# Jackz915/PackPPI

Measured on AMD Instinct MI355X. Metric: sampled residues/sec at 100 diffusion steps, higher is better.
Workload: dtype f32 (dense layers as split-f16: two f16 per operand, three f16 MFMAs per product, fp32 accumulate); 1 GPU; data/T1124_lig.pdb (L=739, 738 true residues), 1 complex per GPU; diffusion_steps=100, proximal=False, residues_per_gpu=738, residues_rank0=738, residues_total=738, mode=ode

## Files before the change

packppi_amd/csrc/pp_api.hip:

```cpp
#include <stdio.h>
#include <stdlib.h>

#include <algorithm>
#include <chrono>
#include <cmath>
#include <cstring>
#include <memory>
#include <new>
#include <string>
#include <vector>

#include "pp_internal.h"
#include "pp_pack.h"
#ifdef PP_EDGE_F16
#include "pp_rebalance.h"
#endif
#include "pp_topk_aten.h"

static thread_local std::string g_err;
void pp_set_error(const std::string &msg) { g_err = msg; }

extern "C" const char *pp_last_error(void) { return g_err.c_str(); }
extern "C" int pp_version(void) { return 101; }
#ifndef PP_BUILD_ID
// ... 310 lines not shown
        if (min_len < PP_TOP_K && min_len != max_len)
            FAIL(PP_ERR_UNSUPPORTED, "pp_complex_prepare_packed: complexes shorter than 32 residues must be prepared on their own");
    }
    if (!b->X || !b->residue_type || !b->BB_D)
        FAIL(PP_ERR_INVALID, "pp_complex_prepare: batch needs at least X, residue_type and BB_D");
    const bool net = plan->has_network;
    if (net && (!b->atom_mask || !b->residue_mask || !b->residue_index || !b->chain_indices || !b->BB_D_sincos ||
                !b->SC_D_mask || !b->chi_1pi_periodic_mask || !b->chi_2pi_periodic_mask))
        FAIL(PP_ERR_INVALID, "pp_complex_prepare: batch has a null tensor pointer");
    PP_HIP_CHECK(hipSetDevice(plan->device));
    std::unique_ptr<pp_ctx, CtxDeleter> owner(new (std::nothrow) pp_ctx());
    if (!owner) FAIL(PP_ERR_INVALID, "out of host memory");
    pp_ctx *c = owner.get();
    c->plan = plan;
    c->b = *b;
    c->packed = packed;
    c->B = packed ? n_seg : b->B;
    c->L = packed ? max_len : b->L;
    c->N = b->B * b->L;
    const int shortest = packed ? min_len : b->L;
    c->K = shortest < PP_TOP_K ? shortest : PP_TOP_K;
    c->shortest = shortest;
    const size_t N = c->N, K = c->K;
    struct Slot { void **p; size_t bytes; };
    std::vector<Slot> slots;
    size_t total = 0;
#define ALLOC(field, n) { const size_t bytes_ = (((n) ? (n) : 1) * sizeof(*c->field) + 255) & ~size_t(255);          \
                          slots.push_back({reinterpret_cast<void **>(&c->field), bytes_}); total += bytes_; }
    if (net) {
        ALLOC(eidx, N * K); ALLOC(mask_att, N * 32); ALLOC(frames, N * 12); ALLOC(bbpos, N * 15);
        ALLOC(hE0, N * K * 128); ALLOC(hE, N * K * 128); ALLOC(Znm, N * K * 128); ALLOC(Zem, N * K * 128); ALLOC(hV, N * 128); ALLOC(hV_alt, N * 128); ALLOC(S, N * 128); ALLOC(msum, N);
        ALLOC(ptsN, N * 48); ALLOC(PAn, N * 128); ALLOC(PCn, N * 128);
        ALLOC(ptsE, N * 48); ALLOC(PAe, N * 128); ALLOC(PCe, N * 128);
        ALLOC(score, N * 4); ALLOC(chi_tmp, N * 4);
        for (int k = 0; k < 2; k++) { ALLOC(live_rows[k], N + 2); ALLOC(live_mix[k], N); ALLOC(live_cnt[k], 1); }
    }
    ALLOC(xyz, N * 42); ALLOC(rec, N * 64); ALLOC(axes, N * 24); ALLOC(rec2, N * 64); ALLOC(axes2, N * 24); ALLOC(brad, N); ALLOC(per_res, N); ALLOC(dchi, N * 4);
    ALLOC(px, N * 4); ALLOC(pm, N * 4); ALLOC(pv, N * 4); ALLOC(pz, N * 4); ALLOC(pxeff, N * 4); ALLOC(pmask, N);
    const bool prox = c->B == 1 || packed;
    if (prox) { ALLOC(cand, (size_t)N * 4 * PP_CL_CAP); ALLOC(cand_cnt, N * 4); }
    ALLOC(scal, 64);
    ALLOC(sat, 4);
    ALLOC(seg, N);
    ALLOC(prox_part, (size_t)PP_PROX_CHUNK * N);
    if (prox) { ALLOC(prox_nrows, c->B); ALLOC(prox_seg, c->B); ALLOC(prox_inv, N); }
    if (prox) { ALLOC(obst_seg, c->B); ALLOC(obst_row, N); ALLOC(obst_cand, (size_t)N * PP_OB_CAP); ALLOC(obst_cnt, N); }
    ALLOC(sasa_row, N * 8);
    ALLOC(seg_off, (size_t)c->B + 1);
    ALLOC(rng_tab, N); ALLOC(rng_keys, c->B);
    c->max_steps = 1 << 20;
#undef ALLOC
    c->last_stream = static_cast<hipStream_t>(stream);
    {
        std::lock_guard<std::mutex> g(plan->pool_mutex);
        int best = -1;
        for (int i = 0; i < (int)plan->arena_pool.size(); i++)
            if (plan->arena_pool[i].bytes >= total && (best < 0 || plan->arena_pool[i].bytes < plan->arena_pool[best].bytes)) best = i;
        if (best >= 0) {
            const ArenaSlot sl = plan->arena_pool[best];
            plan->arena_pool.erase(plan->arena_pool.begin() + best);
            if (sl.stream != c->last_stream) (void)hipStreamSynchronize(sl.stream);
            c->arena = sl.p;
            c->arena_bytes = sl.bytes;
        }
    }
    if (!c->arena && hipMalloc(&c->arena, total) != hipSuccess) {
        c->arena = nullptr;
// ... 654 lines not shown
```

packppi_amd/csrc/pp_internal.h:

```cpp
#pragma once
#include <hip/hip_runtime.h>
#include <hip/hip_ext.h>
#include <cmath>
#include <vector>
#include <mutex>
#include <stdint.h>
#include <string>

#include "../../include/packppi_hip.h"

#if defined(PP_LAB) && !defined(PP_DIAG)
#define PP_DIAG
#endif
#if !defined(PP_LAB) &&                                                                                                       \
    (defined(PP_X_TS) || defined(PP_X_TS_FINE) || defined(PP_X_NOWLOAD) || defined(PP_X_E_NOMFMA) || defined(PP_X_NOSAT) ||      \
     defined(PP_WDEPTH) || defined(PP_WDEPTH_R1) || defined(PP_NXB_R1) || defined(PP_WGS2) || defined(PP_WGS) ||                 \
     defined(PP_NM_WGS2) ||                                                                                                  \
     defined(PP_LDS_PAD) || defined(PP_NO_FUSE_NM) || defined(PP_NU_DEPTH))
#error "PP_X_* / tuning switches compile laboratory variants (most give wrong results): add -DPP_LAB and build a TAGGED library (python -m packppi_amd.build --tag NAME -DPP_LAB -DPP_X_...)"
#endif
#ifdef PP_DIAG
#define PP_GETENV(name) getenv(name)
#else
#define PP_GETENV(name) ((const char *)nullptr)
// ... 76 lines not shown

struct StepParams {
    float temb[16];
    float c_ode;
    float w;
    float c_drift;
    float c_diff;
    float pad[12];
};

struct pp_ctx {
    pp_plan *plan;
    pp_batch b;
    int B, L, K, N;
    bool packed = false;
    int shortest = 0;
    int32_t *seg_off;
    int2 *seg;
    int32_t *eidx;
    float *mask_att;
    float *frames;
    float *bbpos;
    float *hE0;
    float *Znm, *Zem;
    float *hE;
    float *hV;
    float *hV_alt;
    float *S;
    float *msum;
    float *ptsN, *PAn, *PCn;
    float *ptsE, *PAe, *PCe;
    float *score;
    float *chi_tmp;
    void *arena = nullptr;
    size_t arena_bytes = 0;
    hipStream_t last_stream = nullptr;
    int max_steps;
    float *xyz;
    float *rec;
    float *axes;
    float *rec2, *axes2;
    float *brad;
    float *per_res;
    float *dchi;
    float *px, *pm, *pv, *pz, *pxeff;
    uint8_t *pmask;
    int32_t *cand;
    int32_t *cand_cnt;
    float *prox_part;
    int32_t *prox_nrows;
    float2 *prox_seg;
    float *prox_inv;
    float *scal;
    float4 *obst = nullptr;
    int obst_M = 0;
    int obst_cap = 0;
    int2 *obst_seg;
    int2 *obst_row;
    int32_t *obst_cand;
    int32_t *obst_cnt;
    float *sasa_row;
    pp_rng_row *rng_tab;
    uint64_t *rng_keys;
    bool rng_tab_set = false;
    int32_t *live_rows[2];
    int2 *live_mix[2];
// ... 134 lines not shown
    float *chi;
    int step, mode;
    const float *noise;
    const StepParams *cur;
    const StepParams *next;
    const PPRng *rng;
    const PPPin *pin;
};
pp_status pp_launch_node_update(pp_ctx *c, int layer, int last_mode, const NodeEval &ev, hipStream_t s);
pp_status pp_launch_edge_static(pp_ctx *c, hipStream_t s);
#ifdef PP_EDGE_F16
pp_status pp_launch_edge_embed_f16(pp_ctx *c, hipStream_t s);
#endif
pp_status pp_launch_node_message(pp_ctx *c, int layer, hipStream_t s);
bool pp_edge_fused();
pp_status pp_launch_edge_update(pp_ctx *c, int layer, bool keep_hE, hipStream_t s, const PPLive *live = nullptr);
pp_status pp_launch_atom14(pp_ctx *c, const float *chi, float *xyz, hipStream_t s);
pp_status pp_launch_clash(pp_ctx *c, const float *xyz, float *per_res, float *dchi, hipStream_t s, bool use_candidates = false);
pp_status pp_launch_proximal(pp_ctx *c, const float *chi, float lamda, int nsteps, float *traj,
                             float *chi_last, float *losses, hipStream_t s);
pp_status pp_launch_proximal_packed(pp_ctx *c, const float *chi, float lamda, int nsteps, bool norm_given, float *traj,
                                    float *chi_last, float *chi_accepted, float *losses, hipStream_t s,
                                    const uint8_t *fixed = nullptr, uint8_t *moved = nullptr);

pp_status pp_launch_guide_begin(pp_ctx *c, hipStream_t s);
pp_status pp_launch_guide_nudge(pp_ctx *c, float *chi, const uint8_t *fixed, float eta, float cap, double *trace, int n_schedule,
                                int j, hipStream_t s);

pp_status pp_launch_correct(pp_ctx *c, float *chi, const uint8_t *fixed, float snr, int j, int n_steps, const PPRng &rng,
                            double *trace, hipStream_t s);

void pp_edge_occupancy(int *node_msg, int *edge_upd);

#define PP_NU_MID 0
#define PP_NU_SCORE 1
#define PP_NU_STEP 2
```

packppi_amd/csrc/pp_node.hip:

```cpp
#include <string.h>

#include "pp_internal.h"
#include <utility>

PP_RANGE_COUNTER
PP_RANGE_READER(pp_node_range_hits)

#define NT 512
#ifndef PP_NODE_GROUPS
#define PP_NODE_GROUPS 1
#endif
#define NG PP_NODE_GROUPS
#define NB (4 * NG)

struct NodeArgs {
    int N;
    const float *rmask;
    const int64_t *rtype;
    const float *bb_sincos;
    const float *sc_mask;
    const uint8_t *m1pi, *m2pi;
    const float *frames;
    const float *embT, *emb_b, *emb_g, *emb_beta;
    float *hV, *S, *msum;
// ... 278 lines not shown
};

struct SmemU {
    _Float16 a_hi[16 * NU_S128], a_lo[16 * NU_S128];
    _Float16 b_hi[16 * NU_S128], b_lo[16 * NU_S128];
    _Float16 c_hi[16 * NU_S512], c_lo[16 * NU_S512];
    float stats[3][8][16][2];
    float pts[16][48];
    _Float16 e_hi[16 * NU_S32], e_lo[16 * NU_S32];
    float fr[16][12];
    float par[NU_P_LAST_TOTAL];
};

struct StepScalars {
    float c_ode, w, c_drift, c_diff;
};
struct TimeEmb {
    float v[16];
};

struct NUpdArgs {
    int N;
    const float *rmask;
    const int64_t *rtype;
    const float *bb_sincos;
    const float *sc_mask;
    const uint8_t *m1pi, *m2pi;
    const float *frames;
    const float *embT;
    const float *wstream, *params;
    const float *hV;
    float *hV_out;
    const float *S, *msum;
    float *ptsN, *PAn, *PCn, *ptsE, *PAe, *PCe, *score;
    unsigned *sat;
};

template <bool LAST>
__device__ constexpr int nu_slot_waves(int s) {
    if (!LAST) return s < 52 ? 8 : 3;
    return s < 36 ? 8 : s < 40 ? 4 : s < 46 ? 1 : s < 55 ? 8 : 2;
}

template <int CL>
__device__ __forceinline__ int nu_phys_slot(int s, int q) {
    if constexpr (CL == 1) return s;
    constexpr int NPS = 16 / CL;
    return s < 36 ? s : s < 36 + NPS ? s + NPS * q : s + (16 - NPS);
}
template <bool LAST, int CL>
__device__ constexpr int nu_logical_waves(int s) {
    if (CL == 1) return nu_slot_waves<LAST>(s);
    return s < 36 + 16 / CL ? 8 : 3;
}
__device__ __forceinline__ void gload_N(const nh8 *__restrict__ wq, int slot, AOpN &a) {
    int off = slot * 128;
    asm volatile("" : "+s"(off));
    const nh8 *p = wq + off;
    a.hi = p[0];
    a.lo = p[64];
}
#define MFMA_N(a, b, c) __builtin_amdgcn_mfma_f32_16x16x32_f16((a), (b), (c), 0, 0, 0)
__device__ __forceinline__ void mm3(const AOpN &a, const nh8 &bh, const nh8 &bl, nf4 &cH, nf4 &cL) {
    cH = MFMA_N(a.hi, bh, cH);
    cL = MFMA_N(a.hi, bl, cL);
    cL = MFMA_N(a.lo, bh, cL);
}
__device__ __forceinline__ nf4 fold(const nf4 &cH, const nf4 &cL) {
    return nf4{fmaf(cL[0], NU_INV_LO, cH[0]), fmaf(cL[1], NU_INV_LO, cH[1]), fmaf(cL[2], NU_INV_LO, cH[2]), fmaf(cL[3], NU_INV_LO, cH[3])};
}
__device__ __forceinline__ void ldB(const _Float16 *hi, const _Float16 *lo, int rowoff, int ks, nh8 &bh, nh8 &bl) {
    bh = *reinterpret_cast<const nh8 *>(hi + rowoff + 32 * ks);
    bl = *reinterpret_cast<const nh8 *>(lo + rowoff + 32 * ks);
}
__device__ __forceinline__ void split2(float x0, float x1, unsigned &hp, unsigned &lp) {
    unsigned a, b, c, d;
    float fa, fb;
    PP_RANGE(x0) PP_RANGE(x1)
    asm("v_cvt_f16_f32 %0, %1" : "=v"(a) : "v"(x0));
    asm("v_cvt_f16_f32 %0, %1" : "=v"(b) : "v"(x1));
    asm("v_cvt_f32_f16 %0, %1" : "=v"(fa) : "v"(a));
    asm("v_cvt_f32_f16 %0, %1" : "=v"(fb) : "v"(b));
    const float d0 = (x0 - fa) * PP_NU_LO_SCALE, d1 = (x1 - fb) * PP_NU_LO_SCALE;
    asm("v_cvt_f16_f32 %0, %1" : "=v"(c) : "v"(d0));
    asm("v_cvt_f16_f32 %0, %1" : "=v"(d) : "v"(d1));
    asm("v_pack_b32_f16 %0, %1, %2" : "=v"(hp) : "v"(a), "v"(b));
    asm("v_pack_b32_f16 %0, %1, %2" : "=v"(lp) : "v"(c), "v"(d));
// ... 14 lines not shown
}
__device__ __forceinline__ float xsum_g(float v) {
    v += __shfl_xor(v, 16);
    v += __shfl_xor(v, 32);
    return v;
}
__device__ __forceinline__ nf4 ln128(float (*st)[16][2], int wv, int r, int g, const nf4 &x, const nf4 &gain, const nf4 &beta) {
    const float mw = xsum_g((x[0] + x[1]) + (x[2] + x[3])) * (1.f / 16.f);
    const nf4 d = x - mw;
    const float qw = xsum_g(fmaf(d[0], d[0], d[1] * d[1]) + fmaf(d[2], d[2], d[3] * d[3]));
    if (g == 0) *reinterpret_cast<nf2 *>(st[wv][r]) = nf2{mw, qw};
    __syncthreads();
    float m8[8], msum = 0.f, qsum = 0.f;
#pragma unroll
    for (int v = 0; v < 8; v++) {
        const nf2 t = *reinterpret_cast<const nf2 *>(st[v][r]);
        m8[v] = t[0];
        msum += t[0];
        qsum += t[1];
    }
    const float mean = msum * 0.125f;
    float dm = 0.f;
#pragma unroll
    for (int v = 0; v < 8; v++) dm = fmaf(m8[v] - mean, m8[v] - mean, dm);
    const float var = fmaf(16.f, dm, qsum) * (1.f / 128.f);
    const float rstd = 1.f / sqrtf(var + 1e-5f);
    return (x - mean) * rstd * gain + beta;
}

#define NSTAGE_IF(k, OWN, ACCV, BODY)                                                                                  \
    {                                                                                                                  \
        __builtin_amdgcn_sched_barrier(0);                                                                             \
        if constexpr ((k) + NU_ND < NLOAD) {                                                           \
            constexpr int nw_ = nu_logical_waves<LAST, CL>((k) + NU_ND);                                               \
            if (nw_ == 8 || wv < nw_)                                                                                  \
                gload_N(wq, nu_phys_slot<CL>((k) + NU_ND, clq), AR[((k) + NU_ND) % NU_NRING]);                         \
        }                                                                                                              \
        if (OWN) {                                                                                                     \
            const AOpN &AK = AR[(k) % NU_NRING];                                                                       \
            BODY;                                                                                                      \
            asm volatile("" ::"v"(ACCV[0]));                                                                           \
        }                                                                                                              \
    }
#define NSTAGE(k, ACCV, BODY) NSTAGE_IF(k, true, ACCV, BODY)
#define NTILE4_IF(k0, OWN, cH, cL)                                     \
    NSTAGE_IF((k0) + 0, OWN, cH, mm3(AK, bh[0], bl[0], cH, cL))        \
    NSTAGE_IF((k0) + 1, OWN, cH, mm3(AK, bh[1], bl[1], cH, cL))        \
    NSTAGE_IF((k0) + 2, OWN, cH, mm3(AK, bh[2], bl[2], cH, cL))        \
    NSTAGE_IF((k0) + 3, OWN, cH, mm3(AK, bh[3], bl[3], cH, cL))
#define NTILE4(k0, cH, cL) NTILE4_IF(k0, true, cH, cL)
#define LDB4(HI, LO)                                                                  \
    _Pragma("unroll") for (int ks_ = 0; ks_ < 4; ks_++) ldB(HI, LO, r * NU_S128 + 8 * g, ks_, bh[ks_], bl[ks_]);
#define FOSTAGE(s)                                                                                   \
    NSTAGE(20 + (s), cH, {                                                                           \
        if constexpr ((s) + 1 < 16) ldB(sm.c_hi, sm.c_lo, r * NU_S512 + 8 * g, (s) + 1, fh[((s) + 1) & 1], fl[((s) + 1) & 1]); \
        mm3(AK, fh[(s) & 1], fl[(s) & 1], cH, cL);                                                   \
    })

template <int MODE, int NU_ND, int CL = 1, bool SEEDED = false, bool PINNED = false>
__global__ void __launch_bounds__(512)
k_node_update(NUpdArgs A, float *chi, int step, int sde, const float *noise, int embed_next, StepScalars sp, TimeEmb te_next, PPRng rng,
              PPPin pin) {
    static_assert(CL == 1 || MODE == PP_NU_MID, "only the middle layers have a split form");
    static_assert(!SEEDED || MODE == PP_NU_STEP, "only the reverse step draws noise");
    static_assert(!PINNED || SEEDED, "the pinned step is a seeded one: its fixed rows re-noise with the step's own draws");
    constexpr int NU_NRING = NU_ND + 1;
    constexpr bool LAST = MODE != PP_NU_MID;
    constexpr int NSLOT = LAST ? PP_NU_SLOTS_LAST : PP_NU_SLOTS_MID;
    constexpr int NLOAD = MODE == PP_NU_SCORE ? 46 : CL > 1 ? 36 + 16 / CL + 4 : NSLOT;
    const int clq = CL > 1 ? (int)(blockIdx.x % CL) : 0;
    constexpr int NPAR = LAST ? NU_P_LAST_TOTAL : NU_P_MID_TOTAL;
    extern __shared__ __attribute__((aligned(16))) char smem_raw[];
    SmemU &sm = *reinterpret_cast<SmemU *>(smem_raw);
    const int tid = threadIdx.x, lane = tid & 63, wv = __builtin_amdgcn_readfirstlane(tid >> 6);
    const int r = lane & 15, g = lane >> 4, N = A.N, n0 = (int)(blockIdx.x / CL) * 16;
    const int n = n0 + r, nc = n < N ? n : N - 1;
    const bool live = n < N;
    const int fc = 16 * wv + 4 * g;
    const float *par = sm.par;

    const int srow = tid >> 5, scol = (tid & 31) * 4, sn = n0 + srow < N ? n0 + srow : N - 1;
    const nf4 s4 = *reinterpret_cast<const nf4 *>(A.S + (size_t)sn * 128 + scol);
    const nf4 hv4 = *reinterpret_cast<const nf4 *>(A.hV + (size_t)nc * 128 + fc);
    const float ms = A.msum[nc], rm = A.rmask[nc];
    const nf4 zero4i = {0.f, 0.f, 0.f, 0.f};
    float chi1 = 0.f, scm1 = 0.f, nz1 = 0.f, nz2 = 0.f;
    unsigned char m1raw = 0, m2raw = 0;
    int rt = 0;
    pp_rng_row rrow = {0u, 0u, 0u, 0u};
    unsigned char fixraw = 0;
    float cref = 0.f;
    nf4 spv = zero4i;
    if constexpr (MODE == PP_NU_STEP) {
        spv = nf4{sp.c_ode, sp.w, sp.c_drift, sp.c_diff};
        chi1 = chi[(size_t)nc * 4 + g];
        scm1 = A.sc_mask[(size_t)nc * 4 + g];
        m1raw = A.m1pi[(size_t)nc * 4 + g];
        m2raw = A.m2pi[(size_t)nc * 4 + g];
        if constexpr (PINNED) {
            fixraw = pin.fixed[nc];
            cref = pin.chi_ref[(size_t)nc * 4 + g];
        }
        if constexpr (SEEDED) {
            rrow = rng.tab[nc];
        } else if (sde) {
            const size_t NN = (size_t)N * 4;
            const float *nz = noise + (size_t)step * 2 * NN + (size_t)nc * 4 + g;
            nz1 = nz[0];
            nz2 = nz[NN];
        }
        rt = (int)A.rtype[nc];
    }
    nf4 tailv = {0.f, 0.f, 0.f, 0.f};
    nf4 ev[4] = {tailv, tailv, tailv, tailv};
    const int erow = tid & 15, ern = n0 + erow < N ? n0 + erow : N - 1;
    const bool e_bb = MODE == PP_NU_STEP && tid >= 128 && tid < 144, e_te = MODE == PP_NU_STEP && tid >= 192 && tid < 208;
    {
        const int t48 = tid % 48, row = t48 / 3, rn = n0 + row < N ? n0 + row : N - 1;
        tailv = *reinterpret_cast<const nf4 *>(A.frames + (size_t)rn * 12 + 4 * (t48 - 3 * row));
    }
    nf2 bb0 = {0.f, 0.f}, bb1 = bb0, bb2 = bb0;
    if constexpr (MODE == PP_NU_STEP) {
        const nf2 *bp = reinterpret_cast<const nf2 *>(A.bb_sincos + (size_t)ern * 6);
        bb0 = bp[0]; bb1 = bp[1]; bb2 = bp[2];
    }
    constexpr int NPV = (NPAR / 4 + 511) / 512;
    nf4 pv[NPV];
#pragma unroll
// ... 52 lines not shown
        publish4(sm.e_hi, sm.e_lo, erow * NU_S32 + 16, nf4{ev[0][2], ev[0][3], ev[1][0], ev[1][1]});
        publish4(sm.e_hi, sm.e_lo, erow * NU_S32 + 20, nf4{ev[1][2], ev[1][3], ev[2][0], ev[2][1]});
        publish4(sm.e_hi, sm.e_lo, erow * NU_S32 + 24, nf4{ev[2][2], ev[2][3], ev[3][0], ev[3][1]});
        publish4(sm.e_hi, sm.e_lo, erow * NU_S32 + 28, nf4{ev[3][2], ev[3][3], 0.f, 0.f});
    }
    publish4(sm.a_hi, sm.a_lo, srow * NU_S128 + scol, s4);
    unsigned satrows = 0xffffu;
    if constexpr (MODE == PP_NU_STEP) {
        const unsigned long long bs = __ballot(scm1 != 0.f);
        const unsigned long long br = __ballot(rm != 0.f && (!PINNED || fixraw == 0));
        satrows = (unsigned)((bs | (bs >> 16) | (bs >> 32) | (bs >> 48)) & br & 0xffffull);
    }
    __syncthreads();

    nh8 bh[4], bl[4];
    nf4 cH, cL;
    float satm = 0.f;
    const nf4 zero4 = zero4i;
    LDB4(sm.a_hi, sm.a_lo)
    cH = zero4; cL = zero4;
    NTILE4(0, cH, cL)
    nf4 x = fold(cH, cL) + *reinterpret_cast<const nf4 *>(par + NU_P_OUTB + fc) * ms + hv4;
    const nf4 h1 = ln128(sm.stats[0], wv, r, g, x, *reinterpret_cast<const nf4 *>(par + NU_P_G0 + fc),
                         *reinterpret_cast<const nf4 *>(par + NU_P_B0 + fc));
    publish4(sm.b_hi, sm.b_lo, r * NU_S128 + fc, h1);
    __syncthreads();
    LDB4(sm.b_hi, sm.b_lo)
#define FFN_IN_TILE(c)                                                                                     \
    cH = zero4; cL = zero4;                                                                                \
    NTILE4(4 + 4 * (c), cH, cL)                                                                            \
    publish4(sm.c_hi, sm.c_lo, r * NU_S512 + 16 * (4 * wv + (c)) + 4 * g,                                  \
             relu_sat(fold(cH, cL) + *reinterpret_cast<const nf4 *>(par + NU_P_FIB + 16 * (4 * wv + (c)) + 4 * g), satm));
    FFN_IN_TILE(0) FFN_IN_TILE(1) FFN_IN_TILE(2) FFN_IN_TILE(3)
    const bool satrow = (satrows >> r) & 1u;
    if (!(satm < 65504.f) && satrow) atomicOr(A.sat, 2u);
    __syncthreads();
    nh8 fh[2], fl[2];
    ldB(sm.c_hi, sm.c_lo, r * NU_S512 + 8 * g, 0, fh[0], fl[0]);
    cH = zero4; cL = zero4;
    FOSTAGE(0) FOSTAGE(1) FOSTAGE(2) FOSTAGE(3) FOSTAGE(4) FOSTAGE(5) FOSTAGE(6) FOSTAGE(7)
    FOSTAGE(8) FOSTAGE(9) FOSTAGE(10) FOSTAGE(11) FOSTAGE(12) FOSTAGE(13) FOSTAGE(14) FOSTAGE(15)
    x = fold(cH, cL) + *reinterpret_cast<const nf4 *>(par + NU_P_FOB + fc) + h1;
    const nf4 h2 = ln128(sm.stats[1], wv, r, g, x, *reinterpret_cast<const nf4 *>(par + NU_P_G1 + fc),
                         *reinterpret_cast<const nf4 *>(par + NU_P_B1 + fc)) * rm;
    if (live && clq == 0 && (MODE != PP_NU_STEP || !embed_next)) *reinterpret_cast<nf4 *>(A.hV_out + (size_t)n * 128 + fc) = h2;
    publish4(sm.a_hi, sm.a_lo, r * NU_S128 + fc, h2);
    __syncthreads();
    LDB4(sm.a_hi, sm.a_lo)

    if constexpr (!LAST) {
        constexpr int NPJ = 4 / CL;
#define NU_PROJ(i)                                                                                                     \
        if constexpr ((i) < NPJ) {                                                                                     \
            cH = zero4; cL = zero4;                                                                                    \
            NTILE4(36 + 4 * (i), cH, cL)                                                                               \
            const int pj = NPJ * clq + (i);                                                                            \
            float *dst = pj == 0 ? A.PAe : pj == 1 ? A.PCe : pj == 2 ? A.PAn : A.PCn;                                  \
            nf4 v = fold(cH, cL);                                                                                      \
            if (pj == 0) v = v + *reinterpret_cast<const nf4 *>(par + NU_P_PAE_B + fc);                                \
            else if (pj == 2) v = v + *reinterpret_cast<const nf4 *>(par + NU_P_PAN_B + fc);                           \
            if (live) *reinterpret_cast<nf4 *>(dst + (size_t)n * 128 + fc) = v;                                        \
        }
        NU_PROJ(0) NU_PROJ(1) NU_PROJ(2) NU_PROJ(3)
#undef NU_PROJ
        if (CL > 1 && clq != 0) return;
        cH = zero4; cL = zero4;
        NTILE4_IF(36 + 4 * NPJ, wv < 3, cH, cL)
// ... 27 lines not shown
        __syncthreads();
        const bool w0 = wv == 0;
        {
            nh8 dh[2], dl[2];
            if (w0) {
                ldB(sm.c_hi, sm.c_lo, r * NU_S512 + 8 * g, 0, dh[0], dl[0]);
                ldB(sm.c_hi, sm.c_lo, r * NU_S512 + 8 * g, 1, dh[1], dl[1]);
            }
            nf4 eH = zero4, eL = zero4;
            cH = zero4; cL = zero4;
            NSTAGE_IF(40, w0, cH, mm3(AK, dh[0], dl[0], cH, cL))
            NSTAGE_IF(41, w0, cH, mm3(AK, dh[1], dl[1], cH, cL))
            NSTAGE_IF(42, w0, eH, mm3(AK, dh[0], dl[0], eH, eL))
            NSTAGE_IF(43, w0, eH, mm3(AK, dh[1], dl[1], eH, eL))
            if (w0) {
                publish4(sm.c_hi, sm.c_lo, r * NU_S512 + 64 + 4 * g, relu_sat(fold(cH, cL) + *reinterpret_cast<const nf4 *>(par + NU_P_DB1 + 4 * g), satm));
                publish4(sm.c_hi, sm.c_lo, r * NU_S512 + 80 + 4 * g, relu_sat(fold(eH, eL) + *reinterpret_cast<const nf4 *>(par + NU_P_DB1 + 16 + 4 * g), satm));
                asm volatile("s_waitcnt lgkmcnt(0)" ::: "memory");
                ldB(sm.c_hi, sm.c_lo, r * NU_S512 + 8 * g, 2, dh[0], dl[0]);
            }
            cH = zero4; cL = zero4;
            NSTAGE_IF(44, w0, cH, mm3(AK, dh[0], dl[0], cH, cL))
            if (w0) {
                publish4(sm.c_hi, sm.c_lo, r * NU_S512 + 96 + 4 * g, relu_sat(fold(cH, cL) + *reinterpret_cast<const nf4 *>(par + NU_P_DB2 + 4 * g), satm));
                asm volatile("s_waitcnt lgkmcnt(0)" ::: "memory");
                ldB(sm.c_hi, sm.c_lo, r * NU_S512 + 8 * g, 3, dh[0], dl[0]);
            }
            cH = zero4; cL = zero4;
            NSTAGE_IF(45, w0, cH, mm3(AK, dh[0], dl[0], cH, cL))
        }
        if (w0) {
            if (!(satm < 65504.f) && satrow) atomicOr(A.sat, 2u);
            const nf4 sc = fold(cH, cL) + *reinterpret_cast<const nf4 *>(par + NU_P_DB3);
            if (g == 0 && live) *reinterpret_cast<nf4 *>(A.score + (size_t)n * 4) = sc;
            if constexpr (MODE == PP_NU_STEP) {
                const float s0 = __shfl(sc[0], r), s1 = __shfl(sc[1], r), s2 = __shfl(sc[2], r), s3 = __shfl(sc[3], r);
                const float sg = g == 0 ? s0 : g == 1 ? s1 : g == 2 ? s2 : s3;
                const float sp_c_ode = spv[0], sp_w = spv[1], sp_c_drift = spv[2], sp_c_diff = spv[3];
                const float sw = sg * sp_w;
#define NU_M1ON (PINNED ? m1raw == 1 : m1raw != 0)
                float yk = chi1;
                if (!sde) {
                    if (NU_M1ON || m2raw != 0) yk = chi1 + sp_c_ode * sw;
                } else {
                    if (NU_M1ON) yk = chi1 + (sp_c_drift * sw + sp_c_diff * nz1);
                    if (m2raw != 0) yk = yk + (sp_c_drift * sw + sp_c_diff * nz2);
                }
#undef NU_M1ON
                float y = wrap_pi(yk) * scm1;
                if constexpr (PINNED) {
                    if (m1raw == 2) y = chi1;
                }
                if (live) chi[(size_t)n * 4 + g] = y;
                if constexpr (PINNED) {
                    if (pin.traj != nullptr && live) pin.traj[(size_t)n * 4 + g] = y;
                }
                if (embed_next) {
                    unsigned hp, lp;
                    split2(sinf(y) * scm1, cosf(y) * scm1, hp, lp);
                    *reinterpret_cast<unsigned *>(sm.e_hi + r * NU_S32 + 6 + 2 * g) = hp;
                    *reinterpret_cast<unsigned *>(sm.e_lo + r * NU_S32 + 6 + 2 * g) = lp;
                }
            }
        }
        if constexpr (MODE != PP_NU_STEP) return;
        if (!embed_next) return;
        __syncthreads();
        nh8 eh, el;
        eh = *reinterpret_cast<const nh8 *>(sm.e_hi + r * NU_S32 + 8 * g);
        el = *reinterpret_cast<const nh8 *>(sm.e_lo + r * NU_S32 + 8 * g);
        cH = zero4; cL = zero4;
        NSTAGE(46, cH, mm3(AK, eh, el, cH, cL))
        const nf4 e0 = fold(cH, cL) + (*reinterpret_cast<const nf4 *>(par + NU_P_EMB_B + fc) + oh4);
        const nf4 h0 = ln128(sm.stats[2], wv, r, g, e0, *reinterpret_cast<const nf4 *>(par + NU_P_EMB_G + fc),
                             *reinterpret_cast<const nf4 *>(par + NU_P_EMB_BETA + fc));
        if (live) *reinterpret_cast<nf4 *>(A.hV_out + (size_t)n * 128 + fc) = h0;
        publish4(sm.b_hi, sm.b_lo, r * NU_S128 + fc, h0);
        __syncthreads();
        LDB4(sm.b_hi, sm.b_lo)
        cH = zero4; cL = zero4;
        NTILE4(47, cH, cL)
        if (live) *reinterpret_cast<nf4 *>(A.PAn + (size_t)n * 128 + fc) = fold(cH, cL) + *reinterpret_cast<const nf4 *>(par + NU_P_PAN0_B + fc);
        cH = zero4; cL = zero4;
        NTILE4(51, cH, cL)
        if (live) *reinterpret_cast<nf4 *>(A.PCn + (size_t)n * 128 + fc) = fold(cH, cL);
        if (wv < 2) {
            cH = zero4; cL = zero4;
            NTILE4(55, cH, cL)
            if (fc < 24) {
                const nf4 p = fold(cH, cL) + *reinterpret_cast<const nf4 *>(par + NU_P_PTS0_B + fc);
                *reinterpret_cast<nf4 *>(&sm.pts[r][fc]) = p;
                if (live) *reinterpret_cast<nf4 *>(A.ptsN + (size_t)n * 48 + fc) = p;
            }
        }
        __syncthreads();
        if (tid < 128) {
            const int q = tid >> 4, i = tid & 15, ni = n0 + i;
            if (ni < N) {
                const float *fr = sm.fr[i];
                const float px = sm.pts[i][3 * q], py = sm.pts[i][3 * q + 1], pz = sm.pts[i][3 * q + 2];
#pragma unroll
                for (int rr = 0; rr < 3; rr++)
                    A.ptsN[(size_t)ni * 48 + 24 + 3 * q + rr] = (fr[3 * rr] * px + fr[3 * rr + 1] * py + fr[3 * rr + 2] * pz) + fr[9 + rr];
            }
        }
    }
}

#ifndef PP_EDGE_F16
struct UpdW {
    const float *outT, *out_b;
    const float *g0, *b0, *g1, *b1;
    const float *ffn_inT, *ffn_in_b, *ffn_outT, *ffn_out_b;
    PreW pre_edge, pre_next;
    const float *d0_inT, *d0_in_b, *d0_outT, *d0_out_b, *d2_inT, *d2_in_b, *d2_outT, *d2_out_b;
};

struct WSet {
    float v[32];
};
template <int KL, int DST0 = 0>
// ... 345 lines not shown
}
static PreW make_pre(const pp_plan *p, int layer, bool edge) {
    const LayerOff &o = p->off.layer[layer];
    const LayerT &t = p->lt[layer];
    PreW w;
    w.ptsT = edge ? t.pts_edge_wT : t.pts_node_wT;
    w.pts_b = p->w + (edge ? o.pts_edge_b : o.pts_node_b);
    w.AT = edge ? t.em_A_T : t.nm_A_T;
    w.CT = edge ? t.em_C_T : t.nm_C_T;
    w.in_b = p->w + (edge ? o.em_in_b : o.nm_in_b);
    return w;
}

template <typename F>
struct NuInstance {
    int mode, depth, split;
    bool seeded, pinned;
    F fn;
};
typedef void (*nu_kernel_t)(NUpdArgs, float *, int, int, const float *, int, StepScalars, TimeEmb, PPRng, PPPin);
static const NuInstance<nu_kernel_t> nu_table[] = {
    {PP_NU_STEP, PP_NU_DEPTH_MULTI, 1, false, false, k_node_update<PP_NU_STEP, PP_NU_DEPTH_MULTI>},
    {PP_NU_SCORE, PP_NU_DEPTH_MULTI, 1, false, false, k_node_update<PP_NU_SCORE, PP_NU_DEPTH_MULTI>},
    {PP_NU_MID, PP_NU_DEPTH_MULTI, 1, false, false, k_node_update<PP_NU_MID, PP_NU_DEPTH_MULTI>},
    {PP_NU_STEP, PP_NU_DEPTH, 1, false, false, k_node_update<PP_NU_STEP, PP_NU_DEPTH>},
    {PP_NU_SCORE, PP_NU_DEPTH, 1, false, false, k_node_update<PP_NU_SCORE, PP_NU_DEPTH>},
    {PP_NU_MID, PP_NU_DEPTH, 1, false, false, k_node_update<PP_NU_MID, PP_NU_DEPTH>},
    {PP_NU_STEP, PP_NU_DEPTH_MULTI, 1, true, false, k_node_update<PP_NU_STEP, PP_NU_DEPTH_MULTI, 1, true>},
    {PP_NU_STEP, PP_NU_DEPTH, 1, true, false, k_node_update<PP_NU_STEP, PP_NU_DEPTH, 1, true>},
    {PP_NU_STEP, PP_NU_DEPTH_MULTI, 1, true, true, k_node_update<PP_NU_STEP, PP_NU_DEPTH_MULTI, 1, true, true>},
    {PP_NU_STEP, PP_NU_DEPTH, 1, true, true, k_node_update<PP_NU_STEP, PP_NU_DEPTH, 1, true, true>},
    {PP_NU_MID, PP_NU_DEPTH, 4, false, false, k_node_update<PP_NU_MID, PP_NU_DEPTH, 4>},
    {PP_NU_MID, PP_NU_DEPTH, 2, false, false, k_node_update<PP_NU_MID, PP_NU_DEPTH, 2>},
};
#ifndef PP_EDGE_F16
typedef void (*nv_kernel_t)(NodeArgs, UpdW, float *, int, int, const float *, int, PreW, StepScalars, TimeEmb, PPRng, PPPin);
static const NuInstance<nv_kernel_t> nv_table[] = {
    {PP_NU_MID, 0, 1, false, false, k_node_update_valu<PP_NU_MID>},
    {PP_NU_STEP, 0, 1, false, false, k_node_update_valu<PP_NU_STEP>},
    {PP_NU_SCORE, 0, 1, false, false, k_node_update_valu<PP_NU_SCORE>},
    {PP_NU_STEP, 0, 1, true, false, k_node_update_valu<PP_NU_STEP, true>},
    {PP_NU_STEP, 0, 1, true, true, k_node_update_valu<PP_NU_STEP, true, true>},
};
#endif
template <typename F, size_t n>
static F nu_find(const NuInstance<F> (&tab)[n], int mode, int depth, int split, bool seeded, bool pinned) {
    for (const NuInstance<F> &k : tab)
        if (k.mode == mode && k.depth == depth && k.split == split && k.seeded == seeded && k.pinned == pinned) return k.fn;
    return nullptr;
}
static int g_nu_cus = 0;
static pp_status node_attrs() {
    static bool done = false;
    if (!done) {
        PP_HIP_CHECK(hipFuncSetAttribute(reinterpret_cast<const void *>(k_node_embed),
                                         hipFuncAttributeMaxDynamicSharedMemorySize, (int)sizeof(Smem)));
        PP_HIP_CHECK(hipFuncSetAttribute(reinterpret_cast<const void *>(k_node_embed_rows),
                                         hipFuncAttributeMaxDynamicSharedMemorySize, (int)sizeof(Smem)));
        for (const auto &k : nu_table)
            PP_HIP_CHECK(hipFuncSetAttribute(reinterpret_cast<const void *>(k.fn), hipFuncAttributeMaxDynamicSharedMemorySize, (int)sizeof(SmemU)));
#ifndef PP_EDGE_F16
        for (const auto &k : nv_table)
            PP_HIP_CHECK(hipFuncSetAttribute(reinterpret_cast<const void *>(k.fn), hipFuncAttributeMaxDynamicSharedMemorySize, (int)sizeof(Smem)));
#endif
        int dev = 0;
        hipDeviceProp_t prop;
        if (hipGetDevice(&dev) == hipSuccess && hipGetDeviceProperties(&prop, dev) == hipSuccess) g_nu_cus = prop.multiProcessorCount;
        if (g_nu_cus <= 0) g_nu_cus = 256;
        done = true;
    }
    return PP_OK;
}

pp_status pp_launch_node_embed(pp_ctx *c, const float *chi, const StepParams &sp, hipStream_t s) {
    pp_status st = node_attrs();
    if (st != PP_OK) return st;
    NodeArgs A = make_args(c);
    PreW pre0 = make_pre(c->plan, 0, false);
    PP_LAUNCH(c, k_node_embed, dim3((c->N + NB - 1) / NB), dim3(NT), sizeof(Smem), s, A, pre0, chi, sp);
    PP_HIP_CHECK(hipGetLastError());
    return PP_OK;
}

pp_status pp_launch_node_embed_rows(pp_ctx *c, const float *chi, const float *t_rows, hipStream_t s) {
    pp_status st = node_attrs();
    if (st != PP_OK) return st;
    NodeArgs A = make_args(c);
    PreW pre0 = make_pre(c->plan, 0, false);
    TimeFreq fq;
    const float nemb = (float)(-(log(10000.0) / 7.0));
    for (int i = 0; i < 8; i++) fq.v[i] = expf((float)i * nemb);
    hipLaunchKernelGGL(k_node_embed_rows, dim3((c->N + NB - 1) / NB), dim3(NT), sizeof(Smem), s, A, pre0, chi, t_rows, fq);
    PP_HIP_CHECK(hipGetLastError());
    return PP_OK;
}

pp_status pp_launch_node_update(pp_ctx *c, int layer, int last_mode, const NodeEval &ev, hipStream_t s) {
    float *const chi = ev.chi;
    const int step = ev.step;
    const float *const noise = ev.noise;
    const StepParams *cur = last_mode != PP_NU_MID ? ev.cur : nullptr, *next = last_mode == PP_NU_STEP ? ev.next : nullptr;
    const bool pinned = ev.pin != nullptr && last_mode == PP_NU_STEP;
    if (pinned && (ev.rng == nullptr || ev.rng->tab == nullptr || ev.pin->fixed == nullptr || ev.pin->chi_ref == nullptr)) {
        pp_set_error("pp_launch_node_update: the pinned reverse step needs the rng table, fixed and chi_ref");
        return PP_ERR_INVALID;
    }
    const bool seeded = ev.rng != nullptr && ev.rng->tab != nullptr && last_mode == PP_NU_STEP && (ev.mode == PP_MODE_SDE || pinned);
    const PPRng rg = seeded ? *ev.rng : PPRng{nullptr, 0u, 0u};
    const PPPin pn = pinned ? *ev.pin : PPPin{nullptr, nullptr, nullptr, 0.f, 0};
    pp_status st0 = node_attrs();
    if (st0 != PP_OK) return st0;
    if ((last_mode == PP_NU_MID) != (layer < 2)) {
        pp_set_error("pp_launch_node_update: layers 0 and 1 are middle layers, layer 2 is the last one");
// ... 25 lines not shown
    TimeEmb te = {};
    if (cur) sp = {cur->c_ode, cur->w, cur->c_drift, cur->c_diff};
    if (next) memcpy(te.v, next->temb, sizeof(te.v));
#ifndef PP_EDGE_F16
    {
        static const bool f16_node = PP_GETENV("PP_NODE_F16") != nullptr;
        if (!f16_node) {
            const LayerOff &o = p->off.layer[layer];
            NodeArgs NA = make_args(c);
            UpdW W;
            W.outT = t.nm_out_T; W.out_b = p->w + o.nm_out_b;
            W.g0 = p->w + o.norm_g[0]; W.b0 = p->w + o.norm_b[0];
            W.g1 = p->w + o.norm_g[1]; W.b1 = p->w + o.norm_b[1];
            W.ffn_inT = t.nd_in_T; W.ffn_in_b = p->w + o.nd_in_b;
            W.ffn_outT = t.nd_out_T; W.ffn_out_b = p->w + o.nd_out_b;
            W.pre_edge = make_pre(p, layer, true);
            W.pre_next = make_pre(p, layer < 2 ? layer + 1 : 0, false);
            W.d0_inT = p->d0_in_T; W.d0_in_b = p->w + p->off.d0_in_b;
            W.d0_outT = p->d0_out_T; W.d0_out_b = p->w + p->off.d0_out_b;
            W.d2_inT = p->d2_in_T; W.d2_in_b = p->w + p->off.d2_in_b;
            W.d2_outT = p->d2_out_T; W.d2_out_b = p->w + p->off.d2_out_b;
            const PreW pre0 = make_pre(p, 0, false);
            const dim3 vgrid((c->N + NB - 1) / NB), vblock(NT);
            const nv_kernel_t kv = nu_find(nv_table, last_mode, 0, 1, seeded, pinned);
            if (!kv) FAIL(PP_ERR_UNSUPPORTED, "pp_launch_node_update: no such instance of k_node_update_valu");
            PP_LAUNCH(c, kv, vgrid, vblock, sizeof(Smem), s, NA, W, chi, step, sde, noise, embed_next, pre0, sp, te, rg, pn);
            PP_HIP_CHECK(hipGetLastError());
            return PP_OK;
        }
    }
#endif
    const bool multi = (int)grid.x > g_nu_cus;
    static const char *split_env = PP_GETENV("PP_NU_SPLIT");
    static const int split_max = split_env ? atoi(split_env) : 4;
    const int tiles = (int)grid.x;
    const int cl = last_mode != PP_NU_MID ? 1 : (split_max >= 4 && 4 * tiles <= g_nu_cus) ? 4 : (split_max >= 2 && 2 * tiles <= g_nu_cus) ? 2 : 1;
    if (cl > 1) {
        A.hV_out = c->hV_alt;
        std::swap(c->hV, c->hV_alt);
    }
    const nu_kernel_t kern = nu_find(nu_table, last_mode, cl > 1 || !multi ? PP_NU_DEPTH : PP_NU_DEPTH_MULTI, cl, seeded, pinned);
    if (!kern) FAIL(PP_ERR_UNSUPPORTED, "pp_launch_node_update: no such instance of k_node_update");
    PP_LAUNCH(c, kern, dim3(tiles * cl), block, sizeof(SmemU), s, A, chi, step, sde, noise, embed_next, sp, te, rg, pn);
    PP_HIP_CHECK(hipGetLastError());
    return PP_OK;
}

__global__ void k_rng_table(pp_rng_row *__restrict__ tab, int N, const int32_t *__restrict__ seg_off, int n_seg,
                            const uint64_t *__restrict__ keys) {
    const int n = blockIdx.x * blockDim.x + threadIdx.x;
    if (n >= N) return;
    const int ord = pp_seg_of_row(seg_off, n_seg, n);
    const int start = pp_seg_start(seg_off, ord, n);
    const uint64_t key = keys ? keys[ord] : (uint64_t)ord;
    pp_rng_row t;
    t.row = (uint32_t)(n - start);
    t.pad = 0u;
    t.ckey_lo = (uint32_t)key;
    t.ckey_hi = (uint32_t)(key >> 32);
    tab[n] = t;
}

__global__ void k_noise_seeded(const pp_rng_row *__restrict__ tab, int N, uint32_t seed_lo, uint32_t seed_hi, int step,
                               float *__restrict__ noise, uint32_t *__restrict__ words) {
    const int i = blockIdx.x * blockDim.x + threadIdx.x;
    if (i >= N * 4) return;
    const pp_rng_words w = pp_rng_draw(seed_lo, seed_hi, tab[i >> 2], i & 3, step);
    noise[i] = pp_rng_normal(w.o[0], w.o[1]);
    noise[(size_t)N * 4 + i] = pp_rng_normal(w.o[2], w.o[3]);
    if (words) *reinterpret_cast<uint4 *>(words + (size_t)i * 4) = make_uint4(w.o[0], w.o[1], w.o[2], w.o[3]);
}

// ... 118 lines not shown
```

Before: 63780 residues/s.

## Split the reverse-step node update across 2 or 3 workgroups per tile

Extends the cluster-split form of the node-update kernel, previously limited to middle layers, to the final reverse-step kernel. Each tile is replicated 2 or 3 ways: all copies recompute the common trunk, and the trailing projections (PAn, PCn, point heads) are divided among the copies. Only copy 0 writes chi, score and hV. Because several copies read chi while copy 0 writes it, chi is read from a double-buffered snapshot, with a device-to-device copy to seed it. The aim is to fill idle CUs when there are few tiles (L=738), at the cost of redundant trunk compute and extra memory traffic.

```diff
diff --git a/packppi_amd/csrc/pp_api.hip b/packppi_amd/csrc/pp_api.hip
--- a/packppi_amd/csrc/pp_api.hip
+++ b/packppi_amd/csrc/pp_api.hip
@@ -366,7 +366,7 @@
         ALLOC(hE0, N * K * 128); ALLOC(hE, N * K * 128); ALLOC(Znm, N * K * 128); ALLOC(Zem, N * K * 128); ALLOC(hV, N * 128); ALLOC(hV_alt, N * 128); ALLOC(S, N * 128); ALLOC(msum, N);
         ALLOC(ptsN, N * 48); ALLOC(PAn, N * 128); ALLOC(PCn, N * 128);
         ALLOC(ptsE, N * 48); ALLOC(PAe, N * 128); ALLOC(PCe, N * 128);
-        ALLOC(score, N * 4); ALLOC(chi_tmp, N * 4);
+        ALLOC(score, N * 4); ALLOC(chi_tmp, N * 4); ALLOC(chi_snap, N * 8);
         for (int k = 0; k < 2; k++) { ALLOC(live_rows[k], N + 2); ALLOC(live_mix[k], N); ALLOC(live_cnt[k], 1); }
     }
     ALLOC(xyz, N * 42); ALLOC(rec, N * 64); ALLOC(axes, N * 24); ALLOC(rec2, N * 64); ALLOC(axes2, N * 24); ALLOC(brad, N); ALLOC(per_res, N); ALLOC(dchi, N * 4);
diff --git a/packppi_amd/csrc/pp_internal.h b/packppi_amd/csrc/pp_internal.h
--- a/packppi_amd/csrc/pp_internal.h
+++ b/packppi_amd/csrc/pp_internal.h
@@ -132,6 +132,9 @@
     float *ptsE, *PAe, *PCe;
     float *score;
     float *chi_tmp;
+    float *chi_snap;
+    int chi_snap_cur = -1;
+    const float *chi_snap_of = nullptr;
     void *arena = nullptr;
     size_t arena_bytes = 0;
     hipStream_t last_stream = nullptr;
@@ -332,6 +335,4 @@
 
 void pp_edge_occupancy(int *node_msg, int *edge_upd);
 
-#define PP_NU_MID 0
-#define PP_NU_SCORE 1
-#define PP_NU_STEP 2
+#include "pp_nu_split.h"
diff --git a/packppi_amd/csrc/pp_node.hip b/packppi_amd/csrc/pp_node.hip
--- a/packppi_amd/csrc/pp_node.hip
+++ b/packppi_amd/csrc/pp_node.hip
@@ -334,27 +334,14 @@
     const float *hV;
     float *hV_out;
     const float *S, *msum;
-    float *ptsN, *PAn, *PCn, *ptsE, *PAe, *PCe, *score;
+    float *ptsN, *PAn, *PCn;
+    union { float *ptsE; const float *chi_in; };
+    union { float *PAe; float *chi_snap; };
+    float *PCe, *score;
     unsigned *sat;
 };
 
-template <bool LAST>
-__device__ constexpr int nu_slot_waves(int s) {
-    if (!LAST) return s < 52 ? 8 : 3;
-    return s < 36 ? 8 : s < 40 ? 4 : s < 46 ? 1 : s < 55 ? 8 : 2;
-}
-
-template <int CL>
-__device__ __forceinline__ int nu_phys_slot(int s, int q) {
-    if constexpr (CL == 1) return s;
-    constexpr int NPS = 16 / CL;
-    return s < 36 ? s : s < 36 + NPS ? s + NPS * q : s + (16 - NPS);
-}
-template <bool LAST, int CL>
-__device__ constexpr int nu_logical_waves(int s) {
-    if (CL == 1) return nu_slot_waves<LAST>(s);
-    return s < 36 + 16 / CL ? 8 : 3;
-}
+static_assert(PP_NU_STREAM_MID == PP_NU_SLOTS_MID && PP_NU_STREAM_LAST == PP_NU_SLOTS_LAST, "pp_nu_split.h describes these streams");
 __device__ __forceinline__ void gload_N(const nh8 *__restrict__ wq, int slot, AOpN &a) {
     int off = slot * 128;
     asm volatile("" : "+s"(off));
@@ -435,9 +422,9 @@
     {                                                                                                                  \
         __builtin_amdgcn_sched_barrier(0);                                                                             \
         if constexpr ((k) + NU_ND < NLOAD) {                                                           \
-            constexpr int nw_ = nu_logical_waves<LAST, CL>((k) + NU_ND);                                               \
+            constexpr int nw_ = nu_logical_waves<MODE, CL>((k) + NU_ND);                                               \
             if (nw_ == 8 || wv < nw_)                                                                                  \
-                gload_N(wq, nu_phys_slot<CL>((k) + NU_ND, clq), AR[((k) + NU_ND) % NU_NRING]);                         \
+                gload_N(wq, nu_phys_slot<MODE, CL>((k) + NU_ND, clq), AR[((k) + NU_ND) % NU_NRING]);                   \
         }                                                                                                              \
         if (OWN) {                                                                                                     \
             const AOpN &AK = AR[(k) % NU_NRING];                                                                       \
@@ -464,13 +451,14 @@
 __global__ void __launch_bounds__(512)
 k_node_update(NUpdArgs A, float *chi, int step, int sde, const float *noise, int embed_next, StepScalars sp, TimeEmb te_next, PPRng rng,
               PPPin pin) {
-    static_assert(CL == 1 || MODE == PP_NU_MID, "only the middle layers have a split form");
+    static_assert(nu_split_exists(MODE, CL), "the middle layers split 2 or 4 ways, the reverse step 2 or 3 ways");
     static_assert(!SEEDED || MODE == PP_NU_STEP, "only the reverse step draws noise");
     static_assert(!PINNED || SEEDED, "the pinned step is a seeded one: its fixed rows re-noise with the step's own draws");
     constexpr int NU_NRING = NU_ND + 1;
     constexpr bool LAST = MODE != PP_NU_MID;
     constexpr int NSLOT = LAST ? PP_NU_SLOTS_LAST : PP_NU_SLOTS_MID;
-    constexpr int NLOAD = MODE == PP_NU_SCORE ? 46 : CL > 1 ? 36 + 16 / CL + 4 : NSLOT;
+    constexpr int NLOAD = nu_logical_slots(MODE, CL);
+    constexpr bool SPLIT_STEP = MODE == PP_NU_STEP && CL > 1;
     const int clq = CL > 1 ? (int)(blockIdx.x % CL) : 0;
     constexpr int NPAR = LAST ? NU_P_LAST_TOTAL : NU_P_MID_TOTAL;
     extern __shared__ __attribute__((aligned(16))) char smem_raw[];
@@ -496,7 +484,7 @@
     nf4 spv = zero4i;
     if constexpr (MODE == PP_NU_STEP) {
         spv = nf4{sp.c_ode, sp.w, sp.c_drift, sp.c_diff};
-        chi1 = chi[(size_t)nc * 4 + g];
+        chi1 = (SPLIT_STEP ? A.chi_in : chi)[(size_t)nc * 4 + g];
         scm1 = A.sc_mask[(size_t)nc * 4 + g];
         m1raw = A.m1pi[(size_t)nc * 4 + g];
         m2raw = A.m2pi[(size_t)nc * 4 + g];
@@ -615,7 +603,7 @@
     publish4(sm.c_hi, sm.c_lo, r * NU_S512 + 16 * (4 * wv + (c)) + 4 * g,                                  \
              relu_sat(fold(cH, cL) + *reinterpret_cast<const nf4 *>(par + NU_P_FIB + 16 * (4 * wv + (c)) + 4 * g), satm));
     FFN_IN_TILE(0) FFN_IN_TILE(1) FFN_IN_TILE(2) FFN_IN_TILE(3)
-    const bool satrow = (satrows >> r) & 1u;
+    const bool satrow = ((satrows >> r) & 1u) && (!SPLIT_STEP || clq == 0);
     if (!(satm < 65504.f) && satrow) atomicOr(A.sat, 2u);
     __syncthreads();
     nh8 fh[2], fl[2];
@@ -709,7 +697,7 @@
         if (w0) {
             if (!(satm < 65504.f) && satrow) atomicOr(A.sat, 2u);
             const nf4 sc = fold(cH, cL) + *reinterpret_cast<const nf4 *>(par + NU_P_DB3);
-            if (g == 0 && live) *reinterpret_cast<nf4 *>(A.score + (size_t)n * 4) = sc;
+            if (g == 0 && live && (!SPLIT_STEP || clq == 0)) *reinterpret_cast<nf4 *>(A.score + (size_t)n * 4) = sc;
             if constexpr (MODE == PP_NU_STEP) {
                 const float s0 = __shfl(sc[0], r), s1 = __shfl(sc[1], r), s2 = __shfl(sc[2], r), s3 = __shfl(sc[3], r);
                 const float sg = g == 0 ? s0 : g == 1 ? s1 : g == 2 ? s2 : s3;
@@ -728,9 +716,13 @@
                 if constexpr (PINNED) {
                     if (m1raw == 2) y = chi1;
                 }
-                if (live) chi[(size_t)n * 4 + g] = y;
+                const bool put = live && (!SPLIT_STEP || clq == 0);
+                if (put) chi[(size_t)n * 4 + g] = y;
+                if constexpr (SPLIT_STEP) {
+                    if (put) A.chi_snap[(size_t)n * 4 + g] = y;
+                }
                 if constexpr (PINNED) {
-                    if (pin.traj != nullptr && live) pin.traj[(size_t)n * 4 + g] = y;
+                    if (pin.traj != nullptr && put) pin.traj[(size_t)n * 4 + g] = y;
                 }
                 if (embed_next) {
                     unsigned hp, lp;
@@ -751,19 +743,30 @@
         const nf4 e0 = fold(cH, cL) + (*reinterpret_cast<const nf4 *>(par + NU_P_EMB_B + fc) + oh4);
         const nf4 h0 = ln128(sm.stats[2], wv, r, g, e0, *reinterpret_cast<const nf4 *>(par + NU_P_EMB_G + fc),
                              *reinterpret_cast<const nf4 *>(par + NU_P_EMB_BETA + fc));
-        if (live) *reinterpret_cast<nf4 *>(A.hV_out + (size_t)n * 128 + fc) = h0;
+        if (live && (!SPLIT_STEP || clq == 0)) *reinterpret_cast<nf4 *>(A.hV_out + (size_t)n * 128 + fc) = h0;
         publish4(sm.b_hi, sm.b_lo, r * NU_S128 + fc, h0);
         __syncthreads();
         LDB4(sm.b_hi, sm.b_lo)
-        cH = zero4; cL = zero4;
-        NTILE4(47, cH, cL)
-        if (live) *reinterpret_cast<nf4 *>(A.PAn + (size_t)n * 128 + fc) = fold(cH, cL) + *reinterpret_cast<const nf4 *>(par + NU_P_PAN0_B + fc);
-        cH = zero4; cL = zero4;
-        NTILE4(51, cH, cL)
-        if (live) *reinterpret_cast<nf4 *>(A.PCn + (size_t)n * 128 + fc) = fold(cH, cL);
+        if constexpr (CL == 1) {
+            cH = zero4; cL = zero4;
+            NTILE4(47, cH, cL)
+            if (live) *reinterpret_cast<nf4 *>(A.PAn + (size_t)n * 128 + fc) = fold(cH, cL) + *reinterpret_cast<const nf4 *>(par + NU_P_PAN0_B + fc);
+            cH = zero4; cL = zero4;
+            NTILE4(51, cH, cL)
+            if (live) *reinterpret_cast<nf4 *>(A.PCn + (size_t)n * 128 + fc) = fold(cH, cL);
+        } else if (CL == 2 || clq != 0) {
+            const bool pa = clq == CL - 2;
+            cH = zero4; cL = zero4;
+            NTILE4(47, cH, cL)
+            nf4 v = fold(cH, cL);
+            if (pa) v = v + *reinterpret_cast<const nf4 *>(par + NU_P_PAN0_B + fc);
+            if (live) *reinterpret_cast<nf4 *>((pa ? A.PAn : A.PCn) + (size_t)n * 128 + fc) = v;
+            if (clq != 0) return;
+        }
+        constexpr int PTS0 = CL == 1 ? 55 : CL == 2 ? 51 : 47;
         if (wv < 2) {
             cH = zero4; cL = zero4;
-            NTILE4(55, cH, cL)
+            NTILE4(PTS0, cH, cL)
             if (fc < 24) {
                 const nf4 p = fold(cH, cL) + *reinterpret_cast<const nf4 *>(par + NU_P_PTS0_B + fc);
                 *reinterpret_cast<nf4 *>(&sm.pts[r][fc]) = p;
@@ -1175,6 +1178,12 @@
     {PP_NU_STEP, PP_NU_DEPTH, 1, true, true, k_node_update<PP_NU_STEP, PP_NU_DEPTH, 1, true, true>},
     {PP_NU_MID, PP_NU_DEPTH, 4, false, false, k_node_update<PP_NU_MID, PP_NU_DEPTH, 4>},
     {PP_NU_MID, PP_NU_DEPTH, 2, false, false, k_node_update<PP_NU_MID, PP_NU_DEPTH, 2>},
+    {PP_NU_STEP, PP_NU_DEPTH, 3, false, false, k_node_update<PP_NU_STEP, PP_NU_DEPTH, 3>},
+    {PP_NU_STEP, PP_NU_DEPTH, 3, true, false, k_node_update<PP_NU_STEP, PP_NU_DEPTH, 3, true>},
+    {PP_NU_STEP, PP_NU_DEPTH, 3, true, true, k_node_update<PP_NU_STEP, PP_NU_DEPTH, 3, true, true>},
+    {PP_NU_STEP, PP_NU_DEPTH, 2, false, false, k_node_update<PP_NU_STEP, PP_NU_DEPTH, 2>},
+    {PP_NU_STEP, PP_NU_DEPTH, 2, true, false, k_node_update<PP_NU_STEP, PP_NU_DEPTH, 2, true>},
+    {PP_NU_STEP, PP_NU_DEPTH, 2, true, true, k_node_update<PP_NU_STEP, PP_NU_DEPTH, 2, true, true>},
 };
 #ifndef PP_EDGE_F16
 typedef void (*nv_kernel_t)(NodeArgs, UpdW, float *, int, int, const float *, int, PreW, StepScalars, TimeEmb, PPRng, PPPin);
@@ -1222,6 +1231,7 @@
     PreW pre0 = make_pre(c->plan, 0, false);
     PP_LAUNCH(c, k_node_embed, dim3((c->N + NB - 1) / NB), dim3(NT), sizeof(Smem), s, A, pre0, chi, sp);
     PP_HIP_CHECK(hipGetLastError());
+    c->chi_snap_cur = -1;
     return PP_OK;
 }
 
@@ -1313,12 +1323,25 @@
 #endif
     const bool multi = (int)grid.x > g_nu_cus;
     static const char *split_env = PP_GETENV("PP_NU_SPLIT");
-    static const int split_max = split_env ? atoi(split_env) : 4;
+    static const int split_max = split_env ? atoi(split_env) : PP_NU_SPLIT_NOCAP;
     const int tiles = (int)grid.x;
-    const int cl = last_mode != PP_NU_MID ? 1 : (split_max >= 4 && 4 * tiles <= g_nu_cus) ? 4 : (split_max >= 2 && 2 * tiles <= g_nu_cus) ? 2 : 1;
+    const int cl = nu_split_cl(last_mode, tiles, g_nu_cus, split_max, embed_next != 0);
     if (cl > 1) {
         A.hV_out = c->hV_alt;
         std::swap(c->hV, c->hV_alt);
+    }
+    if (last_mode == PP_NU_STEP && cl > 1) {
+        const size_t n4 = (size_t)c->N * 4;
+        if (c->chi_snap_cur < 0 || c->chi_snap_of != chi) {
+            PP_HIP_CHECK(hipMemcpyAsync(c->chi_snap, chi, n4 * sizeof(float), hipMemcpyDeviceToDevice, s));
+            c->chi_snap_cur = 0;
+            c->chi_snap_of = chi;
+        }
+        A.chi_in = c->chi_snap + n4 * c->chi_snap_cur;
+        A.chi_snap = c->chi_snap + n4 * (c->chi_snap_cur ^ 1);
+        c->chi_snap_cur ^= 1;
+    } else if (last_mode == PP_NU_STEP) {
+        c->chi_snap_cur = -1;
     }
     const nu_kernel_t kern = nu_find(nu_table, last_mode, cl > 1 || !multi ? PP_NU_DEPTH : PP_NU_DEPTH_MULTI, cl, seeded, pinned);
     if (!kern) FAIL(PP_ERR_UNSUPPORTED, "pp_launch_node_update: no such instance of k_node_update");
diff --git a/packppi_amd/csrc/pp_nu_split.h b/packppi_amd/csrc/pp_nu_split.h
--- /dev/null
+++ b/packppi_amd/csrc/pp_nu_split.h
@@ -0,0 +1,68 @@
+#pragma once
+
+#define PP_NU_MID 0
+#define PP_NU_SCORE 1
+#define PP_NU_STEP 2
+
+#define PP_NU_SPLIT_NOCAP 0x7fffffff
+#define PP_NU_COMMON_MID 36
+#define PP_NU_COMMON_STEP 47
+#define PP_NU_STREAM_MID 56
+#define PP_NU_STREAM_LAST 59
+
+constexpr int nu_split_cl(int mode, int tiles, int cus, int split_max, bool embed_next = true) {
+    if (mode == PP_NU_MID) {
+        return (split_max >= 4 && 4 * tiles <= cus) ? 4 : (split_max >= 2 && 2 * tiles <= cus) ? 2 : 1;
+    }
+    if (mode == PP_NU_STEP && embed_next) return (split_max >= 3 && 3 * tiles <= cus) ? 3 : (split_max >= 2 && 2 * tiles <= cus) ? 2 : 1;
+    return 1;
+}
+
+constexpr bool nu_split_exists(int mode, int cl) {
+    return cl == 1 || (mode == PP_NU_MID && (cl == 2 || cl == 4)) || (mode == PP_NU_STEP && (cl == 2 || cl == 3));
+}
+
+constexpr int nu_logical_slots(int mode, int cl) {
+    if (mode == PP_NU_SCORE) return 46;
+    if (mode == PP_NU_MID) return cl == 1 ? PP_NU_STREAM_MID : 36 + 16 / cl + 4;
+    return cl == 1 ? PP_NU_STREAM_LAST : cl == 2 ? 55 : 51;
+}
+
+constexpr int nu_used_slots(int mode, int cl, int q) {
+    if (cl == 1 || mode == PP_NU_SCORE) return nu_logical_slots(mode, cl);
+    if (mode == PP_NU_MID) return 36 + 16 / cl + (q == 0 ? 4 : 0);
+    return cl == 3 ? 51 : q == 0 ? 55 : 51;
+}
+
+template <int MODE, int CL>
+constexpr int nu_phys_slot(int s, int q) {
+    static_assert(nu_split_exists(MODE, CL), "no such split");
+    if constexpr (CL == 1) return s;
+    else if constexpr (MODE == PP_NU_MID) {
+        constexpr int NPS = 16 / CL;
+        return s < 36 ? s : s < 36 + NPS ? s + NPS * q : s + (16 - NPS);
+    } else if constexpr (CL == 3) return s < 47 ? s : s + (q == 0 ? 8 : 4 * q - 4);
+    else return s < 47 ? s : s < 51 ? s + 4 * q : s + 4;
+}
+
+constexpr int nu_stream_waves(bool last, int s) {
+    if (!last) return s < 52 ? 8 : 3;
+    return s < 36 ? 8 : s < 40 ? 4 : s < 46 ? 1 : s < 55 ? 8 : 2;
+}
+
+template <int MODE, int CL>
+constexpr int nu_logical_waves(int s) {
+    if (CL == 1) return nu_stream_waves(MODE != PP_NU_MID, s);
+    if (MODE == PP_NU_MID) return s < 36 + 16 / CL ? 8 : 3;
+    return s < 51 ? nu_stream_waves(true, s < 47 ? s : 47) : 2;
+}
+
+constexpr int nu_role_waves(int mode, int cl, int s, int q) {
+    if (s >= nu_used_slots(mode, cl, q)) return 0;
+    const bool last = mode != PP_NU_MID;
+    if (cl == 1) return nu_stream_waves(last, s);
+    if (mode == PP_NU_MID) return s < 36 + 16 / cl ? 8 : 3;
+    if (s < 47) return nu_stream_waves(true, s);
+    if (cl == 3) return q == 0 ? 2 : 8;
+    return s < 51 ? 8 : 2;
+}
```

Result: no change. 64200 residues/s, median of 6 (+0.6%).
